# gogojjh/M-LOAM

Measured on AMD Instinct MI355X. Metric: scan-to-map residuals+Jacobians/sec (features linearised per second, 5 GN iters/frame), higher is better.
Workload: dtype f32 search/fit + f64 residual/Jacobian/normal equations

## Files before the change

### m-loam_amd/csrc/knn_features_kernel.inc

```
    __shared__ int s_run[(G == 16) ? (W / 16) * 2 * KNN_RUN_WORDS : (W / 8) * 2 * KNN_RUN_WORDS];
    __shared__ double s_pose[PRE ? 8 : 1];
    __shared__ float4 s_nbr[FIT ? ((G == 16) ? (W / 16) * 5 : (W / 8) * 5) : 1];
    const KindL k0 = P.k[0], k1 = P.k[1];
    if constexpr (W != TPB) {
        const arg_i4 c0 = MLH_KIND_COUNTS(k0), c1 = MLH_KIND_COUNTS(k1), d0 = MLH_GRID_DIMS(k0), d1 = MLH_GRID_DIMS(k1), w = MLH_WORDS(P);
        const arg_f4 o0 = MLH_GRID_ORIGIN(k0), o1 = MLH_GRID_ORIGIN(k1);
        typedef unsigned long long u64_;
        const arg_u4 p0{u64_(k0.feat), u64_(k0.covd), u64_(k0.nbr), u64_(k0.corr)}, p1{u64_(k1.feat), u64_(k1.covd), u64_(k1.nbr), u64_(k1.corr)};
        const u64_ ro = u64_(P.rows_out);
        const arg_i4 fw{int(unsigned(ro)), int(unsigned(ro >> 32)), P.pre_rows, P.fit_pad_};
        const arg_f2 gate{P.min_match_sq_dis, P.min_plane_dis};
        const arg_d2 loss{P.huber_delta, P.cov_measurement_trace};
#define MLH_KNN_KINDS_WIDE "s"(p0), "s"(c0), "s"(k0.lanes), "s"(k0.grid.sorted), "s"(k0.grid.raw), "s"(k0.grid.cell_start), "s"(o0), "s"(d0), "s"(p1), "s"(c1), "s"(k1.lanes), \
                           "s"(k1.grid.sorted), "s"(k1.grid.raw), "s"(k1.grid.cell_start), "s"(o1), "s"(d1), "s"(w)
        if constexpr (PRE == 0) {
            const arg_d4 ip0{P.init_pose[0], P.init_pose[1], P.init_pose[2], P.init_pose[3]};
            const arg_d2 ip1{P.init_pose[4], P.init_pose[5]};
            const double ip2 = P.init_pose[6];
            const double *const pose_b0 = P.pose_b0, *const pose_bn = P.pose_bn;
            asm volatile("; kernel arguments in registers" ::MLH_KNN_KINDS_WIDE, "s"(ip0), "s"(ip1), "s"(ip2), "s"(pose_b0), "s"(pose_bn));
        } else {
            const double *const x_prev = P.x_prev;
            double *const x_next = P.x_next, *const partials = P.partials;
            const int pre_tiles = P.pre_tiles, pre_from_init = P.pre_from_init;
            if constexpr (PRE == 1) {
                const double thre0 = P.thre_b[0];
                const int freeze0 = P.freeze_b[0];
                if constexpr (FIT) asm volatile("; kernel arguments in registers" ::MLH_KNN_KINDS_WIDE, "s"(x_prev), "s"(x_next), "s"(partials), "s"(pre_tiles), "s"(pre_from_init), "s"(thre0), "s"(freeze0), "s"(fw), "s"(gate), "s"(loss));
                else asm volatile("; kernel arguments in registers" ::MLH_KNN_KINDS_WIDE, "s"(x_prev), "s"(x_next), "s"(partials), "s"(pre_tiles), "s"(pre_from_init), "s"(thre0), "s"(freeze0), "s"(fw));
            } else {
                SolverState *const state = P.state;
                HostPublish *const pre_publish = P.pre_publish;
                const unsigned long long pre_publish_seq = P.pre_publish_seq;
                const double pre_thre = P.pre_thre;
                const int pre_freeze = P.pre_freeze;
                if constexpr (FIT) asm volatile("; kernel arguments in registers" ::MLH_KNN_KINDS_WIDE, "s"(x_prev), "s"(x_next), "s"(partials), "s"(pre_tiles), "s"(pre_from_init), "s"(state), "s"(pre_publish),
                                                "s"(pre_publish_seq), "s"(pre_thre), "s"(pre_freeze), "s"(fw), "s"(gate), "s"(loss));
                else asm volatile("; kernel arguments in registers" ::MLH_KNN_KINDS_WIDE, "s"(x_prev), "s"(x_next), "s"(partials), "s"(pre_tiles), "s"(pre_from_init), "s"(state), "s"(pre_publish),
                                  "s"(pre_publish_seq), "s"(pre_thre), "s"(pre_freeze), "s"(fw));
            }
        }
#undef MLH_KNN_KINDS_WIDE
    } else {
        const arg_i4 c0 = MLH_KIND_COUNTS(k0), c1 = MLH_KIND_COUNTS(k1), d0 = MLH_GRID_DIMS(k0), d1 = MLH_GRID_DIMS(k1), w = MLH_WORDS(P);
        const arg_f4 o0 = MLH_GRID_ORIGIN(k0), o1 = MLH_GRID_ORIGIN(k1);
        const int kb0 = P.kb[0];
#define MLH_KNN_KINDS "s"(k0.feat), "s"(k0.nbr), "s"(c0), "s"(k0.lanes), "s"(k0.grid.sorted), "s"(k0.grid.raw), "s"(k0.grid.cell_start), "s"(o0), "s"(d0), "s"(k1.feat), "s"(k1.nbr), \
                      "s"(c1), "s"(k1.lanes), "s"(k1.grid.sorted), "s"(k1.grid.raw), "s"(k1.grid.cell_start), "s"(o1), "s"(d1), "s"(w), "s"(kb0)
        if constexpr (PRE == 0) {
            const arg_d4 ip0{P.init_pose[0], P.init_pose[1], P.init_pose[2], P.init_pose[3]};
            const arg_d2 ip1{P.init_pose[4], P.init_pose[5]};
            const double ip2 = P.init_pose[6];
            const double *const pose_b0 = P.pose_b0, *const pose_bn = P.pose_bn;
            asm volatile("; kernel arguments in registers" ::MLH_KNN_KINDS, "s"(ip0), "s"(ip1), "s"(ip2), "s"(pose_b0), "s"(pose_bn));
        } else {
            const double *const x_prev = P.x_prev;
            double *const x_next = P.x_next, *const partials = P.partials;
            const int pre_tiles = P.pre_tiles, pre_from_init = P.pre_from_init;
            if constexpr (PRE == 1) {
                const double thre0 = P.thre_b[0];
                const int freeze0 = P.freeze_b[0];
                asm volatile("; kernel arguments in registers" ::MLH_KNN_KINDS, "s"(x_prev), "s"(x_next), "s"(partials), "s"(pre_tiles), "s"(pre_from_init), "s"(thre0), "s"(freeze0));
            } else {
                SolverState *const state = P.state;
                HostPublish *const pre_publish = P.pre_publish;
                const unsigned long long pre_publish_seq = P.pre_publish_seq;
                const double pre_thre = P.pre_thre;
                const int pre_freeze = P.pre_freeze;
                asm volatile("; kernel arguments in registers" ::MLH_KNN_KINDS, "s"(x_prev), "s"(x_next), "s"(partials), "s"(pre_tiles), "s"(pre_from_init), "s"(state), "s"(pre_publish),
                             "s"(pre_publish_seq), "s"(pre_thre), "s"(pre_freeze));
            }
        }
#undef MLH_KNN_KINDS
    }
    int m0 = k0.m, m1 = k1.m, ta0 = k0.tiles_a;
    int total = k0.tiles_a + k1.tiles_a;
    if constexpr (DEVM) {
        static_assert(G == 0 && !MB && PRE == 0, "device-side counts: per-kind lanes, one block, no prologue");
        m0 = P.m_dev[0]; m1 = P.m_dev[1];
        const int f0 = W / k0.lanes, f1 = W / k1.lanes;
        ta0 = (m0 + f0 - 1) / f0;
        total = ta0 + (m1 + f1 - 1) / f1;
        if ((int(blockIdx.x) >> 3) >= ((total + 7) >> 3)) return;
    }
    int tile = xcd_tile(total);
    if (tile >= total) return;
    const int kind = tile >= ta0 ? 1 : 0;
    KindL K = pick_kind(kind != 0, k0, k1);
    int own_mode = P.own_mode;
    if constexpr (PRE != 0 && !MB) {
        asm volatile("" : "+s"(K.feat), "+s"(K.nbr), "+s"(K.nbr_stride), "+s"(K.lanes), "+s"(K.grid.sorted), "+s"(K.grid.raw), "+s"(K.grid.cell_start), "+s"(own_mode));
    }
    [[maybe_unused]] uint32_t fit_flags = P.flags;
    [[maybe_unused]] float min_match_sq_dis = P.min_match_sq_dis, min_plane_dis = P.min_plane_dis;
    [[maybe_unused]] double huber_delta = P.huber_delta, cov_measurement_trace = P.cov_measurement_trace;
    [[maybe_unused]] double *rows_out = P.rows_out;
    [[maybe_unused]] int rows_before = 0, rows_made = 0, rows_all = 0;
    if constexpr (FIT) {
        const int qpw = W / ((G == 0) ? K.lanes : G) / 64;
        rows_before = kind ? 4 * k0.tiles_b : 0;
        rows_made = K.tiles_a * qpw;
        rows_all = 4 * K.tiles_b;
        asm volatile("" : "+s"(K.corr), "+s"(K.covd), "+s"(fit_flags), "+s"(min_match_sq_dis), "+s"(min_plane_dis), "+s"(huber_delta), "+s"(cov_measurement_trace), "+s"(rows_out),
                     "+s"(rows_before), "+s"(rows_made), "+s"(rows_all));
    }
    if constexpr (PRE != 0) {
        __shared__ double f_ne[NE_STRIDE], f_cnt2[2], f_scratch[(GN_SUM_THREADS / 32) * 32];
        int pb = 0;
        bool writer = tile == 0;
        if constexpr (MB) {
            const int tk = kind ? tile - ta0 : tile;
            const int lanes = (G == 0) ? K.lanes : G;
            const int f0 = tk * (W / lanes);
            pb = block_of_slot(P.k[kind], P.n_blocks, f0);
            writer = kind == 0 && f0 == P.k[0].blk_start[pb];
        }
        MLH_KSTAGE(6);
        gn_prologue<PRE, MB, W, W != TPB>(P, pb, s_pose, f_ne, f_cnt2, f_scratch);
        MLH_KSTAGE(7);
        if constexpr (PRE == 2) {
            __shared__ double s_chain[8];
            if (threadIdx.x == 0) {
                if (tile == 0) publish_final_pose(P, s_pose);
                double xc[7], out[7];
                for (int i = 0; i < 7; ++i) xc[i] = s_pose[i];
                double cp[7], cc[7];
                for (int i = 0; i < 7; ++i) { cp[i] = P.chain_prev[i]; cc[i] = P.chain_cur[i]; }
                chain_start_pose(xc, cp, cc, out);
                for (int i = 0; i < 7; ++i) s_chain[i] = out[i];
            }
            __syncthreads();
            if (threadIdx.x < 7) s_pose[threadIdx.x] = s_chain[threadIdx.x];
            __syncthreads();
        }
        if (writer && threadIdx.x < 7) P.x_next[7 * pb + threadIdx.x] = s_pose[threadIdx.x];
    }
    if (kind) tile -= ta0;
    const int m_feat = kind ? m1 : m0;
    [[maybe_unused]] int fit_f = 0;
    [[maybe_unused]] float4 fit_fp = make_float4(0.f, 0.f, 0.f, -1.f), fit_cd = make_float4(0.f, 0.f, 0.f, 0.f);
    if constexpr (FIT) {
        const int fpb = W / ((G == 0) ? K.lanes : G);
        fit_f = tile * fpb + int(threadIdx.x);
        if (int(threadIdx.x) < fpb && fit_f < m_feat) {
            fit_fp = K.feat[fit_f];
            if ((fit_flags & MLH_FLAG_WITH_UA) && K.covd) fit_cd = K.covd[fit_f];
        }
    }
    if constexpr (G == 0) {
        if (K.lanes == 8) knn_features_body<8, MB, K10, PRE != 0, WARM, W, FIT>(P, K, kind, own_mode, tile, s_run, s_pose, m_feat, s_nbr);
        else if (!FIT && K.lanes == 32) knn_features_body<32, MB, K10, PRE != 0, WARM, W>(P, K, kind, own_mode, tile, s_run, s_pose, m_feat);
        else knn_features_body<16, MB, K10, PRE != 0, WARM, W, FIT>(P, K, kind, own_mode, tile, s_run, s_pose, m_feat, s_nbr);
    } else {
        knn_features_body<G, MB, K10, PRE != 0, WARM, W, FIT>(P, K, kind, own_mode, tile, s_run, s_pose, m_feat, s_nbr);
    }
    if constexpr (FIT) {
        const int fpb = W / ((G == 0) ? K.lanes : G);
        MLH_STAGE(blockIdx.x, 0);
        __syncthreads();
        MLH_STAGE(blockIdx.x, 1);
        const int wave = int(threadIdx.x) >> 6;
        if (tile == K.tiles_a - 1 && wave == W / 64 - 1) {
            for (int i = int(threadIdx.x) & 63; i < (rows_all - rows_made) * NE_STRIDE; i += 64) rows_out[size_t(rows_before + rows_made) * NE_STRIDE + i] = 0.0;
        }
        if (int(threadIdx.x) >= fpb) return;
        const q4 q{s_pose[3], s_pose[4], s_pose[5], s_pose[6]};
        const d3 t{s_pose[0], s_pose[1], s_pose[2]};
        bool valid = false;
        float coef[6] = {0.f, 0.f, 0.f, 0.f, 0.f, 0.f};
        if (fit_f < m_feat) {
            float4 nbv[5];
#pragma unroll
            for (int j = 0; j < 5; ++j) nbv[j] = s_nbr[int(threadIdx.x) * 5 + j];
            if (fit_fp.w >= 0.f) {
                valid = fit_feature<5, 5>(min_match_sq_dis, min_plane_dis, kind, nbv, coef);
                if (valid && (fit_flags & MLH_FLAG_CHECK_FOV)) {
                    float sx, sy, sz;
                    associate_to_map(q, t, fit_fp, sx, sy, sz);
                    valid = in_laser_fov(q, t, sx, sy, sz);
                }
            }
            Corr c;
#pragma unroll
            for (int i = 0; i < 6; ++i) c.c[i] = valid ? coef[i] : 0.f;
            c.valid = valid ? 1 : 0;
            c.pad = 0;
            K.corr[fit_f] = c;
        }
        MLH_STAGE(blockIdx.x, 2);
        const Lin L = eval_factor(valid, kind, d3{double(fit_fp.x), double(fit_fp.y), double(fit_fp.z)}, coef, valid ? feature_weight_pref(fit_flags, cov_measurement_trace, K, fit_cd) : 0.0, q, t);
        reduce_rows_wave(valid, L, huber_delta, (fit_flags & MLH_FLAG_NO_LOSS) != 0, kind, rows_out + size_t(rows_before + tile * (fpb / 64) + wave) * NE_STRIDE);
        MLH_STAGE(blockIdx.x, 3);
    }
```

### m-loam_amd/csrc/match.hip

```cpp
#include "ctx.hpp"
#include "solve_host.hpp"
#include "match_plan_host.hpp"
#include "dev_math.hpp"
#include "solver_dev.hpp"
#include "p2p_dev.hpp"
#include "kparams.hpp"
#include <hip/hip_ext.h>
#include <cfloat>
#include <cstdlib>

namespace mlh {

#ifdef MLH_STAGE_CLOCK
__device__ unsigned long long g_stage_clk[4096 * 8];
#define MLH_STAGE(tile, i)                                                                   \
    do {                                                                                     \
        asm volatile("s_waitcnt vmcnt(0) lgkmcnt(0)" ::: "memory");                        \
        if (threadIdx.x == 0 && (tile) < 4096) g_stage_clk[(tile) * 8 + (i)] = wall_clock64(); \
    } while (0)
__device__ unsigned long long g_stage_clk_knn[4096 * 8];
#define MLH_KSTAGE(i)                                                                        \
    do {                                                                                     \
        asm volatile("s_waitcnt vmcnt(0) lgkmcnt(0)" ::: "memory");                        \
        if (threadIdx.x == 0 && blockIdx.x < 4096) g_stage_clk_knn[blockIdx.x * 8 + (i)] = wall_clock64(); \
    } while (0)
#else
#define MLH_STAGE(tile, i) do { } while (0)
#define MLH_KSTAGE(i) do { } while (0)
#endif
}
#include "knn_dev.hpp"
#include "reduce_dev.hpp"
namespace mlh {
__device__ __forceinline__ double sqrt_info_of(double trace)
{
    double s = sqrt(1 / trace);
    return s >= 3.0 ? 1.0 : s / 3.0;
}

__device__ __forceinline__ void eval_plane(const d3 &p, const float (&c)[6], double w, const q4 &q, const d3 &t, const double *R, Lin &o)
{
    d3 n{double(c[0]), double(c[1]), double(c[2])};
    double d = double(c[3]);
    d3 lp = qrot(q, p);
    lp.x += t.x; lp.y += t.y; lp.z += t.z;
    double a = (n.x * lp.x + n.y * lp.y + n.z * lp.z) + d;
    o.r = w * a;
    double wr0 = (-n.x) * R[0] + (-n.y) * R[3] + (-n.z) * R[6];
    double wr1 = (-n.x) * R[1] + (-n.y) * R[4] + (-n.z) * R[7];
    double wr2 = (-n.x) * R[2] + (-n.y) * R[5] + (-n.z) * R[8];
    double j0 = wr0 * 0.0 + wr1 * p.z + wr2 * (-p.y);
    double j1 = wr0 * (-p.z) + wr1 * 0.0 + wr2 * p.x;
    double j2 = wr0 * p.y + wr1 * (-p.x) + wr2 * 0.0;
    o.J[0] = w * n.x; o.J[1] = w * n.y; o.J[2] = w * n.z;
    o.J[3] = w * j0; o.J[4] = w * j1; o.J[5] = w * j2;
}

__device__ __forceinline__ void eval_edge(const d3 &p, const float (&c)[6], double w, const q4 &q, const d3 &t, const double *R, Lin &o)
{
    d3 lpa{double(c[0]), double(c[1]), double(c[2])};
    d3 lpb{double(c[3]), double(c[4]), double(c[5])};
    d3 lp = qrot(q, p);
    lp.x += t.x; lp.y += t.y; lp.z += t.z;
    d3 a{lp.x - lpa.x, lp.y - lpa.y, lp.z - lpa.z};
    d3 b{lp.x - lpb.x, lp.y - lpb.y, lp.z - lpb.z};
    d3 nu = cross3(a, b);
    d3 de{lpa.x - lpb.x, lpa.y - lpb.y, lpa.z - lpb.z};
    double nu_n = sqrt(nu.x * nu.x + nu.y * nu.y + nu.z * nu.z);
    double de_n = sqrt(de.x * de.x + de.y * de.y + de.z * de.z);
    o.r = w * nu_n / de_n;
    double k = 1.0 / de_n;
    double n2 = nu.x * nu.x + nu.y * nu.y + nu.z * nu.z;
    double ex = nu.x, ey = nu.y, ez = nu.z;
    if (n2 > 0.0) { double nn = sqrt(n2); ex /= nn; ey /= nn; ez /= nn; }
    ex = k * ex; ey = k * ey; ez = k * ez;
    double eD0 = ex * 0.0 + ey * de.z + ez * (-de.y);
    double eD1 = ex * (-de.z) + ey * 0.0 + ez * de.x;
    double eD2 = ex * de.y + ey * (-de.x) + ez * 0.0;
    double eDR0 = eD0 * R[0] + eD1 * R[3] + eD2 * R[6];
    double eDR1 = eD0 * R[1] + eD1 * R[4] + eD2 * R[7];
    double eDR2 = eD0 * R[2] + eD1 * R[5] + eD2 * R[8];
    double j0 = eDR0 * 0.0 + eDR1 * p.z + eDR2 * (-p.y);
    double j1 = eDR0 * (-p.z) + eDR1 * 0.0 + eDR2 * p.x;
    double j2 = eDR0 * p.y + eDR1 * (-p.x) + eDR2 * 0.0;
    o.J[0] = w * (-eD0); o.J[1] = w * (-eD1); o.J[2] = w * (-eD2);
    o.J[3] = w * j0; o.J[4] = w * j1; o.J[5] = w * j2;
}

__device__ __forceinline__ Lin eval_factor(bool valid, int kind, const d3 &p, const float (&coef)[6], double w, const q4 &q, const d3 &t)
{
    Lin L;
    L.r = 0.0;
#pragma unroll
    for (int i = 0; i < 6; ++i) L.J[i] = 0.0;
    if (valid) {
        double R[9];
        qtorot(q, R);
        if (kind == MLH_SURF) eval_plane(p, coef, w, q, t, R, L);
        else eval_edge(p, coef, w, q, t, R, L);
    }
    return L;
}

__device__ __forceinline__ bool in_laser_fov(const q4 &q, const d3 &t, float sx, float sy, float sz)
{
    d3 zt = qrot(q, d3{0.0, 0.0, 10.0});
    float zx = float(zt.x + t.x), zy = float(zt.y + t.y), zz = float(zt.z + t.z);
    double a0 = t.x - double(sx), a1 = t.y - double(sy), a2 = t.z - double(sz);
    float squared_side1 = float(a0 * a0 + a1 * a1 + a2 * a2);
    float b0 = zx - sx, b1 = zy - sy, b2 = zz - sz;
    float squared_side2 = b0 * b0 + b1 * b1 + b2 * b2;
    float check1 = 100.0f + squared_side1 - squared_side2 - 10.0f * sqrtf(3.0f) * sqrtf(squared_side1);
    float check2 = 100.0f + squared_side1 - squared_side2 + 10.0f * sqrtf(3.0f) * sqrtf(squared_side1);
    return check1 < 0 && check2 > 0;
}

__device__ __forceinline__ int block_of_slot(const KindP &K, int n_blocks, int f)
{
    int b = 0;
    for (int i = 1; i < n_blocks; ++i) if (f >= K.blk_start[i]) b = i;
    return b;
}

__device__ __forceinline__ const double *block_pose(const KParams &P, int b)
{
    return b == 0 ? (P.pose_sel ? P.state->cand : P.state->x) : P.state->xb[b];
}

__device__ __forceinline__ void load_pose(const KParams &P, int b, q4 &q, d3 &t)
{
    if (P.use_init && b == 0) {
        t = d3{P.init_pose[0], P.init_pose[1], P.init_pose[2]};
        q = q4{P.init_pose[3], P.init_pose[4], P.init_pose[5], P.init_pose[6]};
    } else {
        const double *pose = b == 0 ? P.pose_b0 : P.pose_bn + 7 * b;
        t = d3{pose[0], pose[1], pose[2]};
        q = q4{pose[3], pose[4], pose[5], pose[6]};
    }
}

typedef int arg_i4 __attribute__((ext_vector_type(4)));
typedef float arg_f4 __attribute__((ext_vector_type(4)));
typedef float arg_f2 __attribute__((ext_vector_type(2)));
typedef double arg_d2 __attribute__((ext_vector_type(2)));
typedef double arg_d4 __attribute__((ext_vector_type(4)));
typedef unsigned long long arg_u4 __attribute__((ext_vector_type(4)));
#define MLH_KIND_COUNTS(K_) arg_i4{(K_).m, (K_).tiles_a, (K_).tiles_b, (K_).nbr_stride}
#define MLH_WORDS(P_) arg_i4{int((P_).flags), (P_).own_mode, (P_).n_blocks, (P_).use_init}
#define MLH_GRID_ORIGIN(K_) arg_f4{(K_).grid.ox, (K_).grid.oy, (K_).grid.oz, (K_).grid.inv_h}
#define MLH_GRID_DIMS(K_) arg_i4{(K_).grid.nx, (K_).grid.ny, (K_).grid.nz, (K_).grid.n}

__device__ __forceinline__ KindL pick_kind(bool second, const KindL &a, const KindL &b)
{
    KindL k;
    k.feat = second ? b.feat : a.feat;
    k.covd = second ? b.covd : a.covd;
    k.nbr = second ? b.nbr : a.nbr;
    k.corr = second ? b.corr : a.corr;
    k.r_out = second ? b.r_out : a.r_out;
    k.J_out = second ? b.J_out : a.J_out;
    k.m = second ? b.m : a.m;
    k.tiles_a = second ? b.tiles_a : a.tiles_a;
    k.tiles_b = second ? b.tiles_b : a.tiles_b;
    k.nbr_stride = second ? b.nbr_stride : a.nbr_stride;
    k.lanes = second ? b.lanes : a.lanes;
    k.pad_ = 0;
    k.grid.sorted = second ? b.grid.sorted : a.grid.sorted;
    k.grid.raw = second ? b.grid.raw : a.grid.raw;
    k.grid.cell_start = second ? b.grid.cell_start : a.grid.cell_start;
    k.grid.ox = second ? b.grid.ox : a.grid.ox;
    k.grid.oy = second ? b.grid.oy : a.grid.oy;
    k.grid.oz = second ? b.grid.oz : a.grid.oz;
    k.grid.inv_h = second ? b.grid.inv_h : a.grid.inv_h;
    k.grid.nx = second ? b.grid.nx : a.grid.nx;
    k.grid.ny = second ? b.grid.ny : a.grid.ny;
    k.grid.nz = second ? b.grid.nz : a.grid.nz;
    k.grid.n = second ? b.grid.n : a.grid.n;
    return k;
}

__device__ __forceinline__ void associate_to_map(const q4 &q, const d3 &t, const float4 &fp, float &sx, float &sy, float &sz)
{
    d3 w = qrot(q, d3{double(fp.x), double(fp.y), double(fp.z)});
    sx = float(w.x + t.x); sy = float(w.y + t.y); sz = float(w.z + t.z);
}

__device__ __forceinline__ bool owns(const KParams &P, int own_mode, int f, float sx, float sy, float sz)
{
    if (own_mode == 0) return true;
    const int own_mod = P.own_mod, own_rem = P.own_rem;
    const float l0 = P.lo[0], l1 = P.lo[1], l2 = P.lo[2], l3 = P.lo[3], h0 = P.hi[0], h1 = P.hi[1], h2 = P.hi[2], h3 = P.hi[3];
    bool own = !(own_mode & 4) || (f % (own_mod > 1 ? own_mod : 1)) == own_rem;
    const bool in_lo = (((l0 * sx + l1 * sy) + l2 * sz) + l3) >= 0.f, in_hi = (((h0 * sx + h1 * sy) + h2 * sz) + h3) < 0.f;
    own = own && (!(own_mode & 1) || in_lo);
    own = own && (!(own_mode & 2) || in_hi);
    return own;
}
__device__ __forceinline__ bool owns(const KParams &P, int f, float sx, float sy, float sz) { return owns(P, P.own_mode, f, sx, sy, sz); }


#define MLH_STORE_WINNERS(K_, G_, Kd_, f_, gl_, keys_, HAND_, lds_)                                                        \
    do {                                                                                                        \
        unsigned long long kk_ = keys_[0];                                                                      \
        _Pragma("unroll") for (int t_ = 1; t_ < (K_); ++t_) kk_ = ((gl_) == t_ % (G_)) ? keys_[t_] : kk_;      \
        if ((K_) <= (G_)) {                                                                                     \
            if ((gl_) < (K_)) {                                                                                 \
                float4 o_ = make_float4(0.f, 0.f, 0.f, __uint_as_float(0x7f800000u));                           \
                if (kk_ != KEY_INF) {                                                                           \
                    const float4 np_ = (Kd_).grid.raw[(unsigned)kk_];                                           \
                    o_ = make_float4(np_.x, np_.y, np_.z, __uint_as_float((unsigned)(kk_ >> 32)));              \
                }                                                                                               \
                (Kd_).nbr[size_t(f_) * (Kd_).nbr_stride + (gl_)] = o_;                                          \
                if constexpr (HAND_) (lds_)[(gl_)] = o_;                                                        \
            }                                                                                                   \
        } else {                                                                                                \
            _Pragma("unroll") for (int t_ = 0; t_ < (K_); ++t_) {                                               \
                if ((t_ % (G_)) == (gl_)) {                                                                     \
                    const unsigned long long k2_ = keys_[t_];                                                   \
                    float4 o_ = make_float4(0.f, 0.f, 0.f, __uint_as_float(0x7f800000u));                       \
                    if (k2_ != KEY_INF) {                                                                       \
                        const float4 np_ = (Kd_).grid.raw[(unsigned)k2_];                                       \
                        o_ = make_float4(np_.x, np_.y, np_.z, __uint_as_float((unsigned)(k2_ >> 32)));          \
                    }                                                                                           \
                    (Kd_).nbr[size_t(f_) * (Kd_).nbr_stride + t_] = o_;                                         \
                }                                                                                               \
            }                                                                                                   \
        }                                                                                                       \
    } while (0)

template <int K, int G, bool HAND = false>
__device__ __forceinline__ void knn_feature(const KParams &P, const KindL &Kd, int f, float sx, float sy, float sz, int gl, int *lds_run, float4 *lds_nbr = nullptr)
{
    static_assert(!HAND || K <= G, "the hand-over is the one-record-per-lane store's");
    unsigned long long keys[K];
    if constexpr (G == 32) knn_group_bounded<K, 32, true>(Kd.grid, sx, sy, sz, gl, lds_run, 0x7f800000u, keys);
    else if constexpr (G == 16) knn_group16_pruned<K>(Kd.grid, sx, sy, sz, gl, lds_run, keys);
    else knn_group8_pruned<K>(Kd.grid, sx, sy, sz, gl, lds_run, keys);
    MLH_KSTAGE(4);
    MLH_STORE_WINNERS(K, G, Kd, f, gl, keys, HAND, lds_nbr);
    MLH_KSTAGE(5);
}

template <int K, int G, int NREC, bool HAND = false>
__device__ __forceinline__ void knn_feature_warm(const KParams &P, const KindL &Kd, int f, float sx, float sy, float sz, int gl, int *lds_run, const float4 (&old)[NREC],
                                                 float4 *lds_nbr = nullptr)
{
    unsigned bits = 0u;
#pragma unroll
    for (int r = 0; r < NREC; ++r) {
        if (gl + r * G < K) {
            const float dx = old[r].x - sx, dy = old[r].y - sy, dz = old[r].z - sz;
            const float d = knn_sqdist(dx, dy, dz);
            const unsigned bb = (old[r].w < __uint_as_float(0x7f800000u) && d < __uint_as_float(0x7f800000u)) ? __float_as_uint(d) : 0x7f800000u;
            bits = bb > bits ? bb : bits;
        }
    }
    bits = group_max_u32<G>(bits);
    if (bits >= 0x7f800000u) { knn_feature<K, G, HAND>(P, Kd, f, sx, sy, sz, gl, lds_run, lds_nbr); return; }
    unsigned long long keys[K];
    knn_group_bounded<K, G>(Kd.grid, sx, sy, sz, gl, lds_run, bits, keys);
    MLH_KSTAGE(4);
    MLH_STORE_WINNERS(K, G, Kd, f, gl, keys, HAND, lds_nbr);
    MLH_KSTAGE(5);
}

template <int G, bool MB, bool K10, bool PRE, bool WARM, int W = TPB, bool HAND = false>
__device__ __forceinline__ void knn_features_body(const KParams &P, const KindL &K, int kind, int own_mode, int tile, int *s_run, const double *s_pose, int m_feat,
                                                  float4 *s_nbr = nullptr)
{
    constexpr int FPB = W / G;
    constexpr int RUNW = 2 * KNN_RUN_WORDS;
    const int grp = threadIdx.x / G, gl = threadIdx.x % G;
    const int f = tile * FPB + grp;
    MLH_KSTAGE(0);
    if (f >= m_feat) return;
    const float4 fp = K.feat[f];
    if (fp.w < 0.f) return;
    const int b = MB ? block_of_slot(P.k[kind], P.n_blocks, f) : 0;
    constexpr int NREC = WARM ? ((K10 ? 10 : 5) + G - 1) / G : 1;
    float4 old[NREC];
    if constexpr (WARM) {
        const int kq = K10 ? (MB ? P.kb[b] : P.kb[0]) : 5;
#pragma unroll
        for (int r = 0; r < NREC; ++r) {
            old[r] = make_float4(0.f, 0.f, 0.f, __uint_as_float(0x7f800000u));
            if (gl + r * G < kq) old[r] = K.nbr[size_t(f) * K.nbr_stride + gl + r * G];
        }
    }
    q4 q;
    d3 t;
    if constexpr (PRE) {
        t = d3{s_pose[0], s_pose[1], s_pose[2]};
        q = q4{s_pose[3], s_pose[4], s_pose[5], s_pose[6]};
    } else {
        load_pose(P, b, q, t);
    }
    float sx, sy, sz;
    associate_to_map(q, t, fp, sx, sy, sz);
    MLH_KSTAGE(1);
    if (!owns(P, own_mode, f, sx, sy, sz)) return;
    if constexpr (WARM) {
        if (K10 && (MB ? P.kb[b] : P.kb[0]) == 10) knn_feature_warm<10, G, NREC>(P, K, f, sx, sy, sz, gl, s_run + grp * RUNW, old);
        else knn_feature_warm<5, G, NREC, HAND>(P, K, f, sx, sy, sz, gl, s_run + grp * RUNW, old, s_nbr + (HAND ? grp * 5 : 0));
    } else {
        if (K10 && (MB ? P.kb[b] : P.kb[0]) == 10) knn_feature<10, G>(P, K, f, sx, sy, sz, gl, s_run + grp * RUNW);
        else knn_feature<5, G, HAND>(P, K, f, sx, sy, sz, gl, s_run + grp * RUNW, s_nbr + (HAND ? grp * 5 : 0));
    }
}

constexpr int GN_SUM_THREADS = 256;
template <int MODE, bool MB = false, int W = TPB, bool ROWS = false>
__device__ __forceinline__ void gn_prologue(const KParams &P, int b, double *s_pose, double *f_ne, double *f_cnt2, double *f_scratch)
{
    double pose_v = 0.0;
    if (threadIdx.x < 7) {
        if (P.pre_from_init) pose_v = P.init_pose[threadIdx.x];
        else if (MB && P.pre_from_state) pose_v = (b == 0 ? P.state->x : P.state->xb[b])[threadIdx.x];
        else pose_v = P.x_prev[7 * b + threadIdx.x];
    }
    static_assert(W >= GN_SUM_THREADS && W % 64 == 0, "the sum takes the first 256 threads of the workgroup");
    {
        constexpr int NS = GN_SUM_THREADS / 32, U = 12;
        const int c = threadIdx.x & 31, sl = threadIdx.x >> 5;
        const bool sums = W == GN_SUM_THREADS || threadIdx.x < GN_SUM_THREADS;
        int lo0 = 0, n0 = P.pre_tiles, lo1 = 0, n1 = 0;
        if constexpr (MB) {
            lo0 = P.k[0].m > 0 ? P.k[0].blk_start[b] / TPB : 0;
            n0 = P.k[0].m > 0 ? (P.k[0].blk_start[b + 1] + TPB - 1) / TPB - lo0 : 0;
            lo1 = P.k[0].tiles_b + (P.k[1].m > 0 ? P.k[1].blk_start[b] / TPB : 0);
            n1 = P.k[1].m > 0 ? (P.k[0].tiles_b + (P.k[1].blk_start[b + 1] + TPB - 1) / TPB) - lo1 : 0;
            n0 = max(n0, 0); n1 = max(n1, 0);
        }
        const int ntot = sums ? n0 + n1 : 0;
        const double *__restrict__ rec = P.partials;
        double ch[4] = {0.0, 0.0, 0.0, 0.0};
        bool rows4 = false;
        if constexpr (ROWS) rows4 = P.pre_rows == 4;
        if (ROWS && rows4) {
            static_assert(!ROWS || !MB, "wavefront rows: single-block launches only");
            if constexpr (W > GN_SUM_THREADS) {
                constexpr int PARTS = W / GN_SUM_THREADS >= 4 ? 4 : 2, CPP = 4 / PARTS;
                __shared__ double s_ch[4 * GN_SUM_THREADS];
                const int part = threadIdx.x / GN_SUM_THREADS, t8 = threadIdx.x % GN_SUM_THREADS, pc = t8 & 31, psl = t8 >> 5, nall = n0 + n1;
                if (part < PARTS) {
                    double chp[CPP];
#pragma unroll
                    for (int kk = 0; kk < CPP; ++kk) chp[kk] = 0.0;
                    for (int j = psl; j < nall; j += U * NS) {
                        double wv[CPP][U / 4][4];
#pragma unroll
                        for (int kk = 0; kk < CPP; ++kk)
#pragma unroll
                            for (int v = 0; v < U / 4; ++v) {
                                const int jj = j + NS * (part + PARTS * kk + 4 * v);
#pragma unroll
                                for (int w = 0; w < 4; ++w) wv[kk][v][w] = jj < nall ? rec[(size_t(jj) * 4 + w) * NE_STRIDE + pc] : 0.0;
                            }
#pragma unroll
                        for (int kk = 0; kk < CPP; ++kk)
#pragma unroll
                            for (int v = 0; v < U / 4; ++v) chp[kk] += ((wv[kk][v][0] + wv[kk][v][1]) + wv[kk][v][2]) + wv[kk][v][3];
                    }
#pragma unroll
                    for (int kk = 0; kk < CPP; ++kk) s_ch[(part + PARTS * kk) * GN_SUM_THREADS + t8] = chp[kk];
                }
                __syncthreads();
                if (sums) {
#pragma unroll
                    for (int k = 0; k < 4; ++k) ch[k] = s_ch[k * GN_SUM_THREADS + t8];
                }
            } else {
                for (int j = sl; j < ntot; j += U * NS) {
                    double tv[U];
#pragma unroll
                    for (int h = 0; h < U; h += U / 2) {
                        double wv[U / 2][4];
#pragma unroll
                        for (int u = 0; u < U / 2; ++u) {
                            const int jj = j + NS * (h + u);
#pragma unroll
                            for (int w = 0; w < 4; ++w) wv[u][w] = jj < ntot ? rec[(size_t(jj) * 4 + w) * NE_STRIDE + c] : 0.0;
                        }
#pragma unroll
                        for (int u = 0; u < U / 2; ++u) tv[h + u] = ((wv[u][0] + wv[u][1]) + wv[u][2]) + wv[u][3];
                    }
#pragma unroll
                    for (int u = 0; u < U; ++u) ch[u & 3] += tv[u];
                }
            }
        } else {
            for (int j = sl; j < ntot; j += U * NS) {
                double tv[U];
#pragma unroll
                for (int u = 0; u < U; ++u) {
                    const int jj = j + NS * u;
                    const int tile = jj < n0 ? lo0 + jj : lo1 + (jj - n0);
                    tv[u] = jj < ntot ? rec[size_t(tile) * NE_STRIDE + c] : 0.0;
                }
#pragma unroll
                for (int u = 0; u < U; ++u) ch[u & 3] += tv[u];
            }
        }
        if (sums) f_scratch[sl * 32 + c] = (ch[0] + ch[1]) + (ch[2] + ch[3]);
        if (threadIdx.x < 7) s_pose[threadIdx.x] = pose_v;
        __syncthreads();
        if (threadIdx.x < 32) {
            double tsum = 0.0;
#pragma unroll
            for (int q = 0; q < NS; ++q) tsum += f_scratch[q * 32 + c];
            f_ne[c] = tsum;
        }
        __syncthreads();
    }
    if (threadIdx.x < 64) {
        double xo[7];
        gn_finish_wave(f_ne, f_cnt2, s_pose, nullptr, MODE == 2 ? P.pre_thre : P.thre_b[b], MODE == 2 ? P.pre_freeze : P.freeze_b[b], nullptr, f_scratch, xo);
    }
    __syncthreads();
}

__device__ __forceinline__ void publish_final_pose(const KParams &P, const double *s_pose)
{
    for (int i = 0; i < 7; ++i) P.state->x[i] = s_pose[i];
    if (P.pre_publish) {
        for (int i = 0; i < 7; ++i) P.pre_publish->x[i] = s_pose[i];
        publish_seq(P.pre_publish, P.pre_publish_seq);
    }
}

template <int K, int KV>
__device__ __forceinline__ bool fit_feature(float min_match_sq_dis, float min_plane_dis, int kind, const float4 (&v)[KV], float (&coef)[6]);
__device__ __forceinline__ double feature_weight_pref(uint32_t flags, double cov_measurement_trace, const KindL &K, const float4 &cd);

template <int G, bool MB, bool K10, int PRE = 0, bool WARM = false, bool DEVM = false>
__global__ __launch_bounds__(TPB) void knn_features_kernel(KParams P)
{
    constexpr int W = TPB;
    constexpr bool FIT = false;
#include "knn_features_kernel.inc"
}

template <int W, int G, int PRE, bool WARM, bool FIT = false>
__global__ __launch_bounds__(W) void knn_features_wide_kernel(KParams P)
{
    static_assert(W == 512 || W == 1024, "wide workgroups: 512 or 1024 threads");
    static_assert(!FIT || (PRE != 0 && (G == 0 || W / G >= 64)), "the fused form: a prologue in front, whole wavefront rows per workgroup");
    constexpr bool MB = false, K10 = false, DEVM = false;
#include "knn_features_kernel.inc"
}

__global__ __launch_bounds__(TPB) void gn_final_kernel(KParams P)
{
    __shared__ double s_pose[8], f_ne[NE_STRIDE], f_cnt2[2], f_scratch[(GN_SUM_THREADS / 32) * 32];
    gn_prologue<2, false, TPB, true>(P, 0, s_pose, f_ne, f_cnt2, f_scratch);
    if (threadIdx.x == 0) publish_final_pose(P, s_pose);
}

template <int K>
__device__ __forceinline__ bool fit_plane(const float (&ax)[K], const float (&ay)[K], const float (&az)[K], float min_plane_dis, float (&coef)[6])
{
    float nx, ny, nz;
    plane_fit_qr_f<K>(ax, ay, az, nx, ny, nz);
    float nn = sqrtf(nx * nx + ny * ny + nz * nz);
    float negative_OA_dot_norm = 1 / nn;
    float z = nx * nx + ny * ny + nz * nz;
    if (z > 0.f) { float s = sqrtf(z); nx /= s; ny /= s; nz /= s; }
    bool plane_valid = true;
#pragma unroll
    for (int j = 0; j < K; ++j)
        if (fabsf(nx * ax[j] + ny * ay[j] + nz * az[j] + negative_OA_dot_norm) > min_plane_dis) plane_valid = false;
    coef[0] = nx; coef[1] = ny; coef[2] = nz; coef[3] = negative_OA_dot_norm;
    return plane_valid;
}

template <int K>
__device__ __forceinline__ bool fit_line(const float (&ax)[K], const float (&ay)[K], const float (&az)[K], float (&coef)[6])
{
    float cx = 0.f, cy = 0.f, cz = 0.f;
#pragma unroll
    for (int j = 0; j < K; ++j) { cx += ax[j]; cy += ay[j]; cz += az[j]; }
    const float kf = float(K);
    cx /= kf; cy /= kf; cz /= kf;
    float c00 = 0.f, c10 = 0.f, c11 = 0.f, c20 = 0.f, c21 = 0.f, c22 = 0.f;
#pragma unroll
    for (int j = 0; j < K; ++j) {
        float t0 = ax[j] - cx, t1 = ay[j] - cy, t2 = az[j] - cz;
        c00 += t0 * t0; c10 += t1 * t0; c11 += t1 * t1; c20 += t2 * t0; c21 += t2 * t1; c22 += t2 * t2;
    }
    float l0, l1, l2, vx, vy, vz;
    eig3_largest_f(c00, c10, c11, c20, c21, c22, l0, l1, l2, vx, vy, vz);
    coef[0] = 0.1f * vx + cx; coef[1] = 0.1f * vy + cy; coef[2] = 0.1f * vz + cz;
    coef[3] = -0.1f * vx + cx; coef[4] = -0.1f * vy + cy; coef[5] = -0.1f * vz + cz;
    return l2 > 3 * l1;
}

__device__ __forceinline__ double feature_weight(const KParams &P, const KindP &K, int f)
{
    double trace = P.cov_measurement_trace;
    if ((P.flags & MLH_FLAG_WITH_UA)) {
        trace = 0.0;
        if (K.covd) { float4 cd = K.covd[f]; trace = (double(cd.x) + double(cd.y)) + double(cd.z); }
    }
    return sqrt_info_of(trace);
}

__device__ __forceinline__ double feature_weight_pref(uint32_t flags, double cov_measurement_trace, const KindL &K, const float4 &cd)
{
    double trace = cov_measurement_trace;
    if ((flags & MLH_FLAG_WITH_UA)) {
        trace = 0.0;
        if (K.covd) trace = (double(cd.x) + double(cd.y)) + double(cd.z);
    }
    return sqrt_info_of(trace);
}
__device__ __forceinline__ double feature_weight_pref(const KParams &P, const KindL &K, const float4 &cd) { return feature_weight_pref(P.flags, P.cov_measurement_trace, K, cd); }

__device__ __forceinline__ void load_tile_inputs(const KParams &P, const KindP &K, int f, Corr &c, float4 &fp, float4 &cdv)
{
    c = K.corr[f];
    fp = K.feat[f];
    if ((P.flags & MLH_FLAG_WITH_UA) && K.covd) cdv = K.covd[f];
}

template <typename X>
__device__ __forceinline__ void lmc_publish(const KParams &P, const X &x, int done, int overflow, double used_max, int iteration)
{
    publish_pose(P.publish, P.publish_seq, x, done | (overflow ? DONE_OVERFLOWED : 0), fmax(used_max, double(iteration)));
}

__device__ __forceinline__ void block_sum_args(const KParams &P, int b, int total_tiles, SumArgs &sa)
{
    sa.p = P.partials;
    sa.lo[0] = P.k[0].m > 0 ? P.k[0].blk_start[b] / TPB : 0;
    sa.hi[0] = P.k[0].m > 0 ? (P.k[0].blk_start[b + 1] + TPB - 1) / TPB : 0;
    sa.lo[1] = P.k[0].tiles_b + (P.k[1].m > 0 ? P.k[1].blk_start[b] / TPB : 0);
    sa.hi[1] = P.k[0].tiles_b + (P.k[1].m > 0 ? (P.k[1].blk_start[b + 1] + TPB - 1) / TPB : 0);
    if (P.n_blocks == 1) { sa.lo[0] = 0; sa.hi[0] = total_tiles; sa.lo[1] = 0; sa.hi[1] = 0; }
}

template <bool LM, int NT = TPB, bool COV = false>
__device__ __forceinline__ void fused_gn_finish(const KParams &P, int total_tiles)
{
    __shared__ double f_ne[NE_STRIDE], f_cnt2[2], f_scratch[(NT / 32) * 32];
    if (!last_workgroup_arrives(P.ticket, total_tiles)) return;
    MLH_STAGE(4095, 0);
    if (P.use_init && threadIdx.x < 7) P.state->x[threadIdx.x] = P.init_pose[threadIdx.x];
    __syncthreads();
    if constexpr (LM) {
        SumArgs sa;
        sa.p = P.partials;
        sa.lo[0] = 0; sa.hi[0] = total_tiles; sa.lo[1] = 0; sa.hi[1] = 0;
        sum_partials<NT, (NT > 256 ? 21 : 12)>(sa, f_ne, f_cnt2, f_scratch);
        bool exchanged = true;
        if (P.p2p.n_ranks > 1) {
            exchanged = p2p_exchange<NT>(P.p2p, f_ne, NE_STRIDE);
            if (threadIdx.x == 0) { f_cnt2[0] = f_ne[NE_CNT + 1]; f_cnt2[1] = f_ne[NE_CNT + 2]; }
            __syncthreads();
        }
        MLH_STAGE(4095, 1);
        if (threadIdx.x < 64) {
            double xo[7];
            int done = 0;
            [[maybe_unused]] bool fresh = false;
            if (!exchanged) {
#pragma unroll
                for (int i = 0; i < 7; ++i) xo[i] = P.state->x[i];
                done = 1;
                if (threadIdx.x == 0) P.state->done = 1;
            }
            else if (P.finish == TAIL_LM_BEGIN) {
                if (threadIdx.x == 0 && P.lm_expect_done) {
                    P.state->lm_overflow = (P.lm_expect_done > LM_VERDICT_READ && (P.state->lm_overflow || !P.state->done)) ? 1 : 0;
                    P.state->lm_used_max = P.lm_expect_done > LM_VERDICT_READ ? fmax(P.state->lm_used_max, double(P.state->iteration)) : 0.0;
                }
                lm_begin_body_wave(f_ne, f_cnt2, f_scratch, P.state, P.thre_b[0], P.lm_max_it, P.stat, P.lm_min_blocks, xo, done);
                if constexpr (COV) fresh = true;
            }
            else if constexpr (COV) lm_step_body_wave(f_ne, P.state, P.lm_max_it, xo, done, &fresh);
            else lm_step_body_wave(f_ne, P.state, P.lm_max_it, xo, done);
            if constexpr (COV) { if (P.publish && done && exchanged) publish_pose_cov(P.publish, fresh ? f_ne : P.state->ne); }
            if (threadIdx.x == 0) {
                *P.ticket = 0u;
                if (P.publish) lmc_publish(P, xo, done, P.state->lm_overflow, P.state->lm_used_max, P.state->iteration);
            }
        }
        MLH_STAGE(4095, 2);
        return;
    }
    if (P.finish == TAIL_REDUCE) {
// ... 858 lines not shown
```

Measured before the change: 666.7 million.

## Hoist fit-feature loads before GN prologue and overlap weight prep with KNN

Moves the per-feature loads used by the fit stage (feature point and covariance) ahead of the Gauss-Newton prologue so their latency overlaps it. It also computes the feature weight early, through a prep callback inside the KNN body. In the hand-over path, the feature and warm-neighbour loads are issued unconditionally with clamped indices before the early-exit checks. The neighbour store to LDS is restructured so the raw gather completes before both the LDS and global writes. This adds manual waitcnt instructions and asm register pins, which risk extra register pressure or over-waiting.

```diff
diff --git a/m-loam_amd/csrc/knn_features_kernel.inc b/m-loam_amd/csrc/knn_features_kernel.inc
--- a/m-loam_amd/csrc/knn_features_kernel.inc
+++ b/m-loam_amd/csrc/knn_features_kernel.inc
@@ -104,6 +104,16 @@
         asm volatile("" : "+s"(K.corr), "+s"(K.covd), "+s"(fit_flags), "+s"(min_match_sq_dis), "+s"(min_plane_dis), "+s"(huber_delta), "+s"(cov_measurement_trace), "+s"(rows_out),
                      "+s"(rows_before), "+s"(rows_made), "+s"(rows_all));
     }
+    [[maybe_unused]] int fit_f = 0;
+    [[maybe_unused]] float4 fit_fp = make_float4(0.f, 0.f, 0.f, -1.f), fit_cd = make_float4(0.f, 0.f, 0.f, 0.f);
+    if constexpr (FIT) {
+        const int fpb = W / ((G == 0) ? K.lanes : G);
+        fit_f = (kind ? tile - ta0 : tile) * fpb + int(threadIdx.x);
+        if (int(threadIdx.x) < fpb && fit_f < (kind ? m1 : m0)) {
+            fit_fp = K.feat[fit_f];
+            if ((fit_flags & MLH_FLAG_WITH_UA) && K.covd) fit_cd = K.covd[fit_f];
+        }
+    }
     if constexpr (PRE != 0) {
         __shared__ double f_ne[NE_STRIDE], f_cnt2[2], f_scratch[(GN_SUM_THREADS / 32) * 32];
         int pb = 0;
@@ -118,6 +128,7 @@
         MLH_KSTAGE(6);
         gn_prologue<PRE, MB, W, W != TPB>(P, pb, s_pose, f_ne, f_cnt2, f_scratch);
         MLH_KSTAGE(7);
+        if constexpr (FIT) __builtin_amdgcn_s_waitcnt(0x0F70);
         if constexpr (PRE == 2) {
             __shared__ double s_chain[8];
             if (threadIdx.x == 0) {
@@ -137,22 +148,18 @@
     }
     if (kind) tile -= ta0;
     const int m_feat = kind ? m1 : m0;
-    [[maybe_unused]] int fit_f = 0;
-    [[maybe_unused]] float4 fit_fp = make_float4(0.f, 0.f, 0.f, -1.f), fit_cd = make_float4(0.f, 0.f, 0.f, 0.f);
-    if constexpr (FIT) {
-        const int fpb = W / ((G == 0) ? K.lanes : G);
-        fit_f = tile * fpb + int(threadIdx.x);
-        if (int(threadIdx.x) < fpb && fit_f < m_feat) {
-            fit_fp = K.feat[fit_f];
-            if ((fit_flags & MLH_FLAG_WITH_UA) && K.covd) fit_cd = K.covd[fit_f];
-        }
-    }
+    [[maybe_unused]] double fit_w = 0.0;
+    const auto prep = [&]() {
+        if constexpr (FIT) {
+            if (int(threadIdx.x) < W / ((G == 0) ? K.lanes : G)) fit_w = feature_weight_pref(fit_flags, cov_measurement_trace, K, fit_cd);
+        }
+    };
     if constexpr (G == 0) {
-        if (K.lanes == 8) knn_features_body<8, MB, K10, PRE != 0, WARM, W, FIT>(P, K, kind, own_mode, tile, s_run, s_pose, m_feat, s_nbr);
+        if (K.lanes == 8) knn_features_body<8, MB, K10, PRE != 0, WARM, W, FIT>(P, K, kind, own_mode, tile, s_run, s_pose, m_feat, s_nbr, prep);
         else if (!FIT && K.lanes == 32) knn_features_body<32, MB, K10, PRE != 0, WARM, W>(P, K, kind, own_mode, tile, s_run, s_pose, m_feat);
-        else knn_features_body<16, MB, K10, PRE != 0, WARM, W, FIT>(P, K, kind, own_mode, tile, s_run, s_pose, m_feat, s_nbr);
+        else knn_features_body<16, MB, K10, PRE != 0, WARM, W, FIT>(P, K, kind, own_mode, tile, s_run, s_pose, m_feat, s_nbr, prep);
     } else {
-        knn_features_body<G, MB, K10, PRE != 0, WARM, W, FIT>(P, K, kind, own_mode, tile, s_run, s_pose, m_feat, s_nbr);
+        knn_features_body<G, MB, K10, PRE != 0, WARM, W, FIT>(P, K, kind, own_mode, tile, s_run, s_pose, m_feat, s_nbr, prep);
     }
     if constexpr (FIT) {
         const int fpb = W / ((G == 0) ? K.lanes : G);
@@ -188,7 +195,8 @@
             K.corr[fit_f] = c;
         }
         MLH_STAGE(blockIdx.x, 2);
-        const Lin L = eval_factor(valid, kind, d3{double(fit_fp.x), double(fit_fp.y), double(fit_fp.z)}, coef, valid ? feature_weight_pref(fit_flags, cov_measurement_trace, K, fit_cd) : 0.0, q, t);
+        const Lin L = eval_factor(valid, kind, d3{double(fit_fp.x), double(fit_fp.y), double(fit_fp.z)}, coef, valid ? fit_w : 0.0, q, t);
+        MLH_STAGE(blockIdx.x, 4);
         reduce_rows_wave(valid, L, huber_delta, (fit_flags & MLH_FLAG_NO_LOSS) != 0, kind, rows_out + size_t(rows_before + tile * (fpb / 64) + wave) * NE_STRIDE);
         MLH_STAGE(blockIdx.x, 3);
     }
diff --git a/m-loam_amd/csrc/match.hip b/m-loam_amd/csrc/match.hip
--- a/m-loam_amd/csrc/match.hip
+++ b/m-loam_amd/csrc/match.hip
@@ -203,7 +203,19 @@
     do {                                                                                                        \
         unsigned long long kk_ = keys_[0];                                                                      \
         _Pragma("unroll") for (int t_ = 1; t_ < (K_); ++t_) kk_ = ((gl_) == t_ % (G_)) ? keys_[t_] : kk_;      \
-        if ((K_) <= (G_)) {                                                                                     \
+        if (HAND_) {                                                                                            \
+                           \
+            float4 o_ = make_float4(0.f, 0.f, 0.f, __uint_as_float(0x7f800000u));                               \
+            if ((gl_) < (K_) && kk_ != KEY_INF) {                                                               \
+                const float4 np_ = (Kd_).grid.raw[(unsigned)kk_];                                               \
+                o_ = make_float4(np_.x, np_.y, np_.z, __uint_as_float((unsigned)(kk_ >> 32)));                  \
+            }                                                                                                   \
+            __builtin_amdgcn_s_waitcnt(0x0F70);                                                   \
+            if ((gl_) < (K_)) {                                                                                 \
+                (lds_)[(gl_)] = o_;                                                                             \
+                (Kd_).nbr[size_t(f_) * (Kd_).nbr_stride + (gl_)] = o_;                                          \
+            }                                                                                                   \
+        } else if ((K_) <= (G_)) {                                                                              \
             if ((gl_) < (K_)) {                                                                                 \
                 float4 o_ = make_float4(0.f, 0.f, 0.f, __uint_as_float(0x7f800000u));                           \
                 if (kk_ != KEY_INF) {                                                                           \
@@ -211,9 +223,8 @@
                     o_ = make_float4(np_.x, np_.y, np_.z, __uint_as_float((unsigned)(kk_ >> 32)));              \
                 }                                                                                               \
                 (Kd_).nbr[size_t(f_) * (Kd_).nbr_stride + (gl_)] = o_;                                          \
-                if constexpr (HAND_) (lds_)[(gl_)] = o_;                                                        \
             }                                                                                                   \
-        } else {                                                                                                \
+        } else {                                                                                             \
             _Pragma("unroll") for (int t_ = 0; t_ < (K_); ++t_) {                                               \
                 if ((t_ % (G_)) == (gl_)) {                                                                     \
                     const unsigned long long k2_ = keys_[t_];                                                   \
@@ -264,27 +275,41 @@
     MLH_KSTAGE(5);
 }
 
-template <int G, bool MB, bool K10, bool PRE, bool WARM, int W = TPB, bool HAND = false>
+struct NoPrep { __device__ __forceinline__ void operator()() const {} };
+template <int G, bool MB, bool K10, bool PRE, bool WARM, int W = TPB, bool HAND = false, typename PREP = NoPrep>
 __device__ __forceinline__ void knn_features_body(const KParams &P, const KindL &K, int kind, int own_mode, int tile, int *s_run, const double *s_pose, int m_feat,
-                                                  float4 *s_nbr = nullptr)
+                                                  float4 *s_nbr = nullptr, const PREP &prep = PREP())
 {
     constexpr int FPB = W / G;
     constexpr int RUNW = 2 * KNN_RUN_WORDS;
     const int grp = threadIdx.x / G, gl = threadIdx.x % G;
     const int f = tile * FPB + grp;
     MLH_KSTAGE(0);
-    if (f >= m_feat) return;
-    const float4 fp = K.feat[f];
-    if (fp.w < 0.f) return;
-    const int b = MB ? block_of_slot(P.k[kind], P.n_blocks, f) : 0;
     constexpr int NREC = WARM ? ((K10 ? 10 : 5) + G - 1) / G : 1;
-    float4 old[NREC];
-    if constexpr (WARM) {
-        const int kq = K10 ? (MB ? P.kb[b] : P.kb[0]) : 5;
-#pragma unroll
-        for (int r = 0; r < NREC; ++r) {
-            old[r] = make_float4(0.f, 0.f, 0.f, __uint_as_float(0x7f800000u));
-            if (gl + r * G < kq) old[r] = K.nbr[size_t(f) * K.nbr_stride + gl + r * G];
+    float4 fp, old[NREC];
+    int b = 0;
+    if constexpr (HAND) {
+        static_assert(!MB && !K10 && NREC == 1, "the fused form");
+        const int fl = f < m_feat ? f : m_feat - 1;
+        fp = K.feat[fl];
+        if constexpr (WARM) old[0] = K.nbr[size_t(fl) * K.nbr_stride + (gl < 5 ? gl : 4)];
+        prep();
+        asm volatile("" : "+v"(fp.x), "+v"(fp.y), "+v"(fp.z), "+v"(fp.w));
+        if constexpr (WARM) asm volatile("" : "+v"(old[0].x), "+v"(old[0].y), "+v"(old[0].z), "+v"(old[0].w));
+        if (f >= m_feat || fp.w < 0.f) return;
+        if (WARM && gl >= 5) old[0] = make_float4(0.f, 0.f, 0.f, __uint_as_float(0x7f800000u));
+    } else {
+        if (f >= m_feat) return;
+        fp = K.feat[f];
+        if (fp.w < 0.f) return;
+        b = MB ? block_of_slot(P.k[kind], P.n_blocks, f) : 0;
+        if constexpr (WARM) {
+            const int kq = K10 ? (MB ? P.kb[b] : P.kb[0]) : 5;
+#pragma unroll
+            for (int r = 0; r < NREC; ++r) {
+                old[r] = make_float4(0.f, 0.f, 0.f, __uint_as_float(0x7f800000u));
+                if (gl + r * G < kq) old[r] = K.nbr[size_t(f) * K.nbr_stride + gl + r * G];
+            }
         }
     }
     q4 q;
```

Result: no change. 661.5 million (-0.8%).
